# Gyeeta/gyeeta

Measured on NVIDIA H100. Metric: events/sec aggregated, higher is better.
Workload: dtype u64

## Files before the change

gyeeta_b200/csrc/gysk_kernels.cu:

```cuda
#include "gysk_kernels.cuh"
#include "gysk_state.cuh"
#include "gysk_summary.cuh"

#include <cfloat>
#include <climits>
#include <cmath>
#include <algorithm>
#include <type_traits>
#include <cstdlib>
#include <cstring>

namespace gysk {

static constexpr int KEY_GROUP_SHIFT = 30;
static constexpr int KEY_SLOT_SHIFT = KEY_GROUP_SHIFT + TD_CODE_BITS;
__device__ __forceinline__ uint32_t key_usec(unsigned long long k) { return (uint32_t)k & 0x3FFFFFFFu; }
__device__ __forceinline__ uint32_t key_slot(unsigned long long k) { return (uint32_t)(k >> KEY_SLOT_SHIFT); }
__device__ __forceinline__ uint32_t key_bin(unsigned long long k) { return (uint32_t)(k >> KEY_GROUP_SHIFT) & ((1u << TD_CODE_BITS) - 1u); }

static constexpr int KEY_DIGIT_MAX = 8;
struct SortPlan { int np; int shift[OS_MAX_PASSES_VK]; int bits[OS_MAX_PASSES_VK]; int exp; };

__global__ void init_state_kernel(DevState st, uint32_t max_svcs, uint32_t max_tasks)
{
// ... 769 lines not shown
		if (k == ~0ull) return ~0u;
		const uint32_t s = key_slot(k), r1 = s == sf ? rf : (s == sl ? rl : 0u);
		return r1 ? ((r1 - 1u) << TD_CODE_BITS) | key_bin(k) : ~0u;
	};
	auto red_bin = [&](uint32_t d, unsigned long long cw, unsigned long long us) {
		unsigned long long *row = rows + (size_t)(d >> TD_CODE_BITS) * HOT_ROW_WORDS;
		const uint32_t w = hot_word(d & ((1u << TD_CODE_BITS) - 1u));
		red_add_u64(row + w, cw);
		red_add_u64(row + w + HOT_ROW_BINS, us);
	};

	const uint32_t dfirst = __shfl_sync(0xffffffffu, dest(kk[0]), 0), dlast = __shfl_sync(0xffffffffu, dest(kk[LS_V - 1]), 31);
	if (dfirst == dlast && dlast != ~0u) {
		unsigned long long us = 0;
		uint32_t rem = 0;
#pragma unroll
		for (int t = 0; t < LS_V; ++t) { const uint32_t v = key_usec(kk[t]); us += v; rem += v - (v / 1000u) * 1000u; }
		const unsigned long long gsum = (unsigned long long)__reduce_add_sync(0xffffffffu, (uint32_t)us & 0xFFFFFu) +
				((unsigned long long)__reduce_add_sync(0xffffffffu, (uint32_t)(us >> 20)) << 20);
		rem = __reduce_add_sync(0xffffffffu, rem);
		if (lane == 0) red_bin(dlast, (unsigned long long)(32 * LS_V) | ((unsigned long long)rem << BIN_CNT_BITS), gsum);
		return;
	}

	uint32_t pd[LS_V], pc[LS_V], prem[LS_V];
	unsigned long long ps[LS_V];
	bool tail[LS_V];
#pragma unroll
	for (int t = 0; t < LS_V; ++t) {
		const uint32_t d = dest(kk[t]);
		const bool valid = d != ~0u;
		tail[t] = valid;
		const uint32_t v = key_usec(kk[t]);
		pd[t] = valid ? d : (0x80000000u | (uint32_t)lane); pc[t] = valid ? 1u : 0u; ps[t] = valid ? v : 0u; prem[t] = valid ? v - (v / 1000u) * 1000u : 0u;
		if (t > 0 && valid && pd[t] == pd[t - 1]) { pc[t] += pc[t - 1]; ps[t] += ps[t - 1]; prem[t] += prem[t - 1]; tail[t - 1] = false; }
	}
#pragma unroll
	for (int t = 0; t < LS_V; ++t) {
		const bool act = tail[t];
		if (!__any_sync(0xffffffffu, act)) continue;
		const uint32_t did = act ? pd[t] : (0x80000000u | (uint32_t)lane);
		const unsigned long long v = act ? ps[t] : 0ull;
		uint32_t cnt = act ? pc[t] : 0u, rem = act ? prem[t] : 0u;
		const uint32_t m = __match_any_sync(0xffffffffu, did);
		unsigned long long gsum = v;
		const uint32_t maxcnt = __reduce_max_sync(0xffffffffu, (uint32_t)__popc(m));
		uint32_t rest = m & ~(1u << lane);
		const uint32_t cnt0 = cnt, rem0 = rem;
		for (uint32_t u = 1; u < maxcnt; ++u) {
			const int src = rest ? (__ffs(rest) - 1) : lane;
			const unsigned long long ov = __shfl_sync(0xffffffffu, v, src);
			const uint32_t oc = __shfl_sync(0xffffffffu, cnt0, src), orr = __shfl_sync(0xffffffffu, rem0, src);
			if (rest) { gsum += ov; cnt += oc; rem += orr; rest &= rest - 1; }
		}
		if (act && (m & ((1u << lane) - 1u)) == 0) red_bin(did, (unsigned long long)cnt | ((unsigned long long)rem << BIN_CNT_BITS), gsum);
	}
}

__global__ void __launch_bounds__(256) long_sum_kernel(const unsigned long long *__restrict__ keys, const unsigned long long *__restrict__ d_n,
		const BatchSeg *__restrict__ segs, const unsigned long long *__restrict__ nlong, unsigned long long *__restrict__ rows)
{
	if (*nlong == 0) return;
	const uint64_t n = *d_n;
	const uint64_t nchunks = (n + 127) >> 7;
	const int lane = threadIdx.x & 31;
	const uint64_t gw = ((uint64_t)blockIdx.x * blockDim.x + threadIdx.x) >> 5, nwarps = ((uint64_t)gridDim.x * blockDim.x) >> 5;
	for (uint64_t c0 = gw * 32; c0 < nchunks; c0 += nwarps * 32) {
		const uint64_t c = c0 + lane;
		uint32_t sf = 0, sl = 0, rf = 0, rl = 0;
		if (c < nchunks) {
			const uint64_t f = c << 7, l = f + 127 < n ? f + 127 : n - 1;
			sf = key_slot(keys[f]); sl = key_slot(keys[l]);
			rf = segs[sf].row1; rl = segs[sl].row1;
		}
		for (uint32_t todo = __ballot_sync(0xffffffffu, (rf | rl) != 0); todo; todo &= todo - 1) {
			const int src = __ffs(todo) - 1;
			long_sum_chunk(keys, n, (c0 + (uint64_t)src) << 7, __shfl_sync(0xffffffffu, sf, src), __shfl_sync(0xffffffffu, rf, src),
					__shfl_sync(0xffffffffu, sl, src), __shfl_sync(0xffffffffu, rl, src), rows);
		}
	}
}

static constexpr int TD_WARPS = 3;
static constexpr int TD_SMEM_N = 384;

__global__ void __launch_bounds__(TD_WARPS * 32, TD_MERGE_CTAS_PER_SM) bins_merge_kernel(DevState st, const unsigned long long *__restrict__ keys,
		const uint32_t *__restrict__ touched, const unsigned long long *__restrict__ ntouched_p, const uint32_t *__restrict__ long_slot,
		const unsigned long long *__restrict__ nlong_p, unsigned long long *__restrict__ batch_rows, const BatchSeg *__restrict__ segs,
		Centroid *__restrict__ items_scratch , TdWorkBig *__restrict__ big_scratch )
{
	__shared__ TdWorkT<TD_SMEM_N> work[TD_WARPS];
	__shared__ uint32_t hcnt[TD_WARPS][16], hsum_lo[TD_WARPS][16], hsum_hi[TD_WARPS][16];
	__shared__ uint16_t first_idx[16];
	const int lane = threadIdx.x & 31, wid = threadIdx.x >> 5;
	const uint32_t gw = blockIdx.x * TD_WARPS + wid, nwarps = gridDim.x * TD_WARPS;

	Centroid *items = items_scratch + (size_t)gw * NBINS;
	const uint32_t ntouched = (uint32_t)*ntouched_p, nlong = (uint32_t)*nlong_p;

	if (threadIdx.x < 16) {
		constexpr uint32_t thr[13] = {1, 10, 30, 60, 100, 150, 200, 300, 450, 700, 1000, 3000, 15000};
		const uint32_t bk = threadIdx.x;
		const uint32_t first_us = bk < 2 ? 0u : (bk > 14 ? 0u : (thr[bk - 2] + 1u) * 1000u);
		first_idx[bk] = (uint16_t)(bk == 0 ? 0u : (bk > 14 ? 0xFFFFu : td_code(first_us) + bk));
	}
	__syncthreads();

	const uint32_t nhot = st.hot_rows ? (uint32_t)st.counters[CTR_NHOT] : 0u;
	const uint32_t nrow = nhot + nlong, total = nrow + ntouched;
	const uint32_t lt = (1u << lane) - 1u;
	auto slot_of = [&](uint32_t t) { return t < nhot ? st.hot_slot[t] : (t < nrow ? long_slot[t - nhot] : touched[t - nrow]); };
	uint32_t nslot = gw < total ? slot_of(gw) : 0u;
	for (uint32_t t = gw; t < total; t += nwarps) {
		const uint32_t slot = nslot;
		const bool has_next = t + nwarps < total;
		nslot = has_next ? slot_of(t + nwarps) : 0u;
		const SlotBatch sb = st.slot_batch[slot];
		BatchSeg seg {0u, 0u, 0u, 0u};
		if (t >= nrow) seg = segs[slot];
		uint2 nseg = make_uint2(0u, 0u);
		if (has_next) {
			prefetch_l2(st.td_cent + (size_t)nslot * TD_CAP + lane * (TD_CAP / 32));
			if (lane == 0) prefetch_l2(st.slot_batch + nslot);
			else if (lane == 1) prefetch_l2(st.td_head + nslot);
			if (t + nwarps >= nrow) { const BatchSeg ns = segs[nslot]; nseg = make_uint2(ns.key0, ns.end); }
		}
		if (t < nhot && sb.minv == 0xFFFFFFFFu) continue;
		if (lane < 16) { hcnt[wid][lane] = 0; hsum_lo[wid][lane] = 0; hsum_hi[wid][lane] = 0; }
		__syncwarp();
		auto take_bin = [&](uint32_t j, unsigned long long cw, unsigned long long us, uint32_t bin) {
			const unsigned long long cnt = cw & BIN_CNT_MASK, rem = cw >> BIN_CNT_BITS;
			Centroid c; c.mean = __ddiv_rn((double)us, (double)cnt); c.weight = cnt;
			items[j] = c;
			uint32_t bk = 0;
#pragma unroll
			for (int q = 1; q < 15; ++q) bk += bin >= first_idx[q];
			atomicAdd(&hcnt[wid][bk], (uint32_t)cnt);
			const unsigned long long ms = (us - rem) / 1000ull;
			const uint32_t mlo = (uint32_t)ms, mhi = (uint32_t)(ms >> 32);
			const uint32_t old = atomicAdd(&hsum_lo[wid][bk], mlo);
			const uint32_t up = mhi + (old + mlo < old ? 1u : 0u);
			if (up) atomicAdd(&hsum_hi[wid][bk], up);
		};
		uint32_t nitems = 0, nsamples, binmax = 0;
		if (t >= nrow) {
			nsamples = seg.end - seg.key0;
			constexpr int RAW_BIN_SHIFT = 54;
			static_assert(BIN_CNT_BITS + 10 + 14 <= RAW_BIN_SHIFT && LONG_SEG <= (1 << 14), "cw of a short segment's bin below the bin bits");
			ulonglong2 *raw = reinterpret_cast<ulonglong2 *>(items);
			uint32_t pbin = ~0u, ccnt = 0, crem = 0;
			unsigned long long cus = 0;
			for (uint32_t b0 = seg.key0; b0 < seg.end; b0 += 128) {
				uint32_t bin[4], v[4];
#pragma unroll
				for (int u = 0; u < 4; ++u) {
					const uint32_t i = b0 + (uint32_t)u * 32 + lane;
					const unsigned long long k = i < seg.end ? keys[i] : 0ull;
					bin[u] = i < seg.end ? key_bin(k) : ~0u;
					v[u] = key_usec(k);
				}
				const uint32_t xbin = b0 + 128 < seg.end ? key_bin(keys[b0 + 128]) : ~0u;
#pragma unroll
				for (int u = 0; u < 4; ++u) {
					if (b0 + (uint32_t)u * 32 >= seg.end) break;
					uint32_t pb = __shfl_up_sync(0xffffffffu, bin[u], 1), nb = __shfl_down_sync(0xffffffffu, bin[u], 1);
					const uint32_t nb31 = u < 3 ? __shfl_sync(0xffffffffu, bin[u < 3 ? u + 1 : 0], 0) : xbin;
					if (lane == 0) pb = pbin;
					if (lane == 31) nb = nb31;
					const bool valid = bin[u] != ~0u;
					const uint32_t hm = __ballot_sync(0xffffffffu, valid && bin[u] != pb);
					const uint32_t upto = hm & (0xFFFFFFFFu >> (31 - lane));
					const int h = upto ? 31 - __clz((int)upto) : 0;
					const uint32_t r = v[u] - (v[u] / 1000u) * 1000u;
					const uint32_t a = valid ? v[u] & 0xFFFFFu : 0u, b = valid ? (v[u] >> 20) | (r << 16) : 0u;
					uint32_t ai = a, bi = b;
#pragma unroll
					for (int off = 1; off < 32; off <<= 1) {
						const uint32_t x = __shfl_up_sync(0xffffffffu, ai, off), y = __shfl_up_sync(0xffffffffu, bi, off);
						if (lane >= off) { ai += x; bi += y; }
					}
					const uint32_t as = ai - __shfl_sync(0xffffffffu, ai - a, h), bs = bi - __shfl_sync(0xffffffffu, bi - b, h);
					uint32_t cnt = (uint32_t)(lane - h) + 1u, rem = bs >> 16;
					unsigned long long us = (unsigned long long)as + ((unsigned long long)(bs & 0xFFFFu) << 20);
					if (!upto) { cnt += ccnt; rem += crem; us += cus; }
					if (valid && bin[u] != nb) {
						raw[nitems + __popc(upto) - 1u] = make_ulonglong2(us, (unsigned long long)cnt | ((unsigned long long)rem << BIN_CNT_BITS) |
								((unsigned long long)bin[u] << RAW_BIN_SHIFT));
						binmax = max(binmax, cnt);
					}
					ccnt = __shfl_sync(0xffffffffu, cnt, 31); crem = __shfl_sync(0xffffffffu, rem, 31); cus = __shfl_sync(0xffffffffu, us, 31);
					pbin = __shfl_sync(0xffffffffu, bin[u], 31);
					nitems += __popc(hm);
				}
			}
			__syncwarp();
			for (uint32_t j = lane; j < nitems; j += 32) {
				const ulonglong2 r = raw[j];
				take_bin(j, r.y & ((1ull << RAW_BIN_SHIFT) - 1u), r.x, (uint32_t)(r.y >> RAW_BIN_SHIFT));
			}
		}
		else {
			unsigned long long *row = t < nhot ? st.hot_rows + (size_t)t * HOT_ROW_WORDS : batch_rows + (size_t)(t - nhot) * HOT_ROW_WORDS;
			uint32_t mine = 0;
			for (uint32_t b0 = 0; b0 < (uint32_t)NBINS; b0 += 32) {
				const uint32_t bin = b0 + lane;
				const uint32_t i0 = hot_word(bin), i1 = i0 + (uint32_t)HOT_ROW_BINS;
				ulonglong2 v = make_ulonglong2(0ull, 0ull);
				if (bin < (uint32_t)NBINS) { v.x = __ldcg(row + i0); v.y = __ldcg(row + i1); }
				const bool ne = (v.x & BIN_CNT_MASK) != 0;
				const uint32_t m = __ballot_sync(0xffffffffu, ne);
				if (ne) {
					take_bin(nitems + __popc(m & lt), v.x, v.y, bin);
					row[i0] = 0ull; row[i1] = 0ull;
					mine += (uint32_t)(v.x & BIN_CNT_MASK);
					binmax = max(binmax, (uint32_t)(v.x & BIN_CNT_MASK));
				}
				nitems += __popc(m);
			}
			nsamples = __reduce_add_sync(0xffffffffu, mine);
		}
		if (has_next && t + nwarps >= nrow) {
			const uint32_t l0 = nseg.x >> 4, l1 = (nseg.y - 1u) >> 4;
			if (l0 + lane <= l1) prefetch_l2(keys + (size_t)(l0 + lane) * 16);
		}
		binmax = __reduce_max_sync(0xffffffffu, binmax);
		__syncwarp();
		if (lane < HIST_MAX_CELL) {
			if (hcnt[wid][lane]) {
				HistCell *c = st.hist_cur + (size_t)slot * HIST_CELLS + lane;
				c->count += hcnt[wid][lane]; c->sum += (long long)(((unsigned long long)hsum_hi[wid][lane] << 32) | hsum_lo[wid][lane]);
			}
		}
		else if (lane == HIST_MAX_CELL) {
			HistCell *c = st.hist_cur + (size_t)slot * HIST_CELLS + HIST_MAX_CELL;
			const long long mx = (long long)(sb.maxv / 1000u);
			if (mx > c->sum) c->sum = mx;
			uint32_t hot = sb.hot;
			if (!hot && st.hot_rows && nsamples >= st.hot_min && nsamples <= st.hot_max && binmax <= st.hot_bin_max) {
				const unsigned long long h = atomicAdd(st.counters + CTR_NHOT_NEXT, 1ull);
				if (h < (unsigned long long)st.hot_cap) { st.hot_slot[h] = slot; hot = (uint32_t)h + 1u; }
				else atomicAdd(st.counters + CTR_NHOT_NEXT, ~0ull);
			}
			st.slot_batch[slot] = SlotBatch {0xFFFFFFFFu, 0u, 0u, hot};
		}
		__syncwarp();

		TdHead head = st.td_head[slot];
		Centroid *cent = st.td_cent + (size_t)slot * TD_CAP;
		uint32_t nout;
		if (head.n + nitems <= (uint32_t)TD_SMEM_N) nout = warp_merge_compress(work[wid], cent, head.n, items, nitems, cent, st.td);
		else nout = warp_merge_compress(big_scratch[gw], cent, head.n, items, nitems, cent, st.td);
		if (lane == 0) {
			head.n = nout;
			head.total += nsamples;
			if ((double)sb.minv < head.minv) head.minv = (double)sb.minv;
			if ((double)sb.maxv > head.maxv) head.maxv = (double)sb.maxv;
			st.td_head[slot] = head;
		}
		__syncwarp();
	}
}

__global__ void flush_kernel(DevState st, uint32_t nslots, uint32_t tsec, uint32_t idle_secs)
{
	const uint64_t i = (uint64_t)blockIdx.x * blockDim.x + threadIdx.x;
	const bool valid = i < (uint64_t)nslots * HIST_CELLS;
	const int cell = (int)(i & (HIST_CELLS - 1));
	HistCell c {0, 0};
	unsigned long long cc = 0;
	const uint32_t slot = (uint32_t)(i >> 4);

	if (valid) {
		c = st.hist_cur[i];
		if (cell == HIST_MAX_CELL) cc = st.conn_cur[slot];
	}
	bool auxact = false;
	if (valid && cell == HIST_MAX_CELL) { const SlotAux a0 = st.slot_aux[slot]; auxact = (a0.act_cur | a0.err_cur) != 0; }
	const uint32_t bal = __ballot_sync(0xffffffffu, valid && (cell == HIST_MAX_CELL ? (cc != 0 || auxact) : c.count != 0));
	const bool active = ((bal >> (threadIdx.x & 16)) & 0xFFFFu) != 0;
	if (!valid) return;

	st.bm_last[i] = st.bm_cur[i]; st.bm_cur[i] = 0;
	st.hist_last[i] = c;
	HistCell &r0 = st.levels.row(0, st.levels.cur[0], slot)[cell], &r1 = st.levels.row(1, st.levels.cur[1], slot)[cell];
	if (cell == HIST_MAX_CELL) {
		if (c.sum > r0.sum) r0.sum = c.sum;
		if (c.sum > r1.sum) r1.sum = c.sum;
	}
	else {
		r0.count += c.count; r0.sum += c.sum;
		r1.count += c.count; r1.sum += c.sum;
	}
	if (cell == HIST_MAX_CELL) {
		if (c.sum > st.hist_all[i].sum) st.hist_all[i].sum = c.sum;
		st.hist_cur[i].count = 0; st.hist_cur[i].sum = LLONG_MIN;
		st.conn_last[slot] = cc;
		st.conn_all_cnt[slot] += (uint32_t)cc;
		st.conn_all_kb[slot] += cc >> 32;
		st.conn_cur[slot] = 0;
		{
			SlotAux a = st.slot_aux[slot];
			a.act_last = a.act_cur; a.act_cur = 0; a.err_last = a.err_cur; a.err_cur = 0; a.rtt_last = a.rtt_cur; a.rtt_cur = 0;
			st.slot_aux[slot] = a;
		}

		const unsigned long long id = st.slot_id[slot];
		if (id) {
			uint32_t first = st.slot_first_seen[slot], last = st.slot_last_active[slot];
			if (!first) { first = tsec ? tsec : 1u; st.slot_first_seen[slot] = first; }
			if (active) { last = tsec ? tsec : 1u; st.slot_last_active[slot] = last; }
			if (idle_secs && last && (uint64_t)last + idle_secs < tsec && (uint64_t)first + 2ull * idle_secs < tsec) {
				const unsigned long long k = atomicAdd(st.counters + CTR_NEVICT, 1ull);
				st.evict_list[k] = slot;
				st.evict_ids[k] = id;
			}
		}
	}
	else {
		st.hist_all[i].count += c.count;
		st.hist_all[i].sum += c.sum;
		st.hist_cur[i].count = 0; st.hist_cur[i].sum = 0;
	}
}

struct LevelStat { int64_t p95, p99, p25; uint64_t cnt, sum; double mean; };

__device__ __forceinline__ LevelStat level_stat(const uint64_t *counts, uint64_t sum)
{
	LevelStat r;
	uint64_t c = 0;
	for (int b = 0; b < HIST_MAX_CELL; ++b) c += counts[b];
	r.p95 = resp_bucket_value(hist_pct_bucket(counts, HIST_MAX_CELL, c, 95.0f), c);
	r.p99 = resp_bucket_value(hist_pct_bucket(counts, HIST_MAX_CELL, c, 99.0f), c);
	r.p25 = resp_bucket_value(hist_pct_bucket(counts, HIST_MAX_CELL, c, 25.0f), c);
// ... 517 lines not shown
	uint32_t e = ++*tmp.epoch;
	if (e == 0) {
		cudaMemsetAsync(tmp.tile_status, 0, (size_t)max_tiles * RADIX_MAX * sizeof(unsigned long long), s);
		e = ++*tmp.epoch;
	}
	return e;
}

static void launch_os_pass(int bits, uint32_t ntiles, const unsigned long long *in, unsigned long long *out, const unsigned long long *d_n, const DigitSpec &D,
		const uint32_t *ghist, unsigned long long *status, uint32_t *ticket, uint32_t epoch, cudaStream_t s)
{
	const uint32_t grid = std::min<uint32_t>(ntiles, (uint32_t)sm_count(current_device()) * 4u);
	if (bits > 8) os_pass_kernel<9><<<grid, OS_THREADS, sizeof(OneSweepSharedT<9>), s>>>(in, out, d_n, D, ghist, status, ticket, epoch);
	else if (bits == 8) os_pass_kernel<8><<<grid, OS_THREADS, sizeof(OneSweepSharedT<8>), s>>>(in, out, d_n, D, ghist, status, ticket, epoch);
	else if (bits == 7) os_pass_kernel<7><<<grid, OS_THREADS, sizeof(OneSweepSharedT<7>), s>>>(in, out, d_n, D, ghist, status, ticket, epoch);
	else os_pass_kernel<6><<<grid, OS_THREADS, sizeof(OneSweepSharedT<6>), s>>>(in, out, d_n, D, ghist, status, ticket, epoch);
}

int launch_radix_sort(const SortTemp &tmp, const unsigned long long *d_n, uint64_t n_max, int lo1, int hi1, int lo2, int hi2, int *which, cudaStream_t s)
{
	int launches = 0;
	unsigned long long *bufs[2] = { tmp.keys_a, tmp.keys_b };
	int w = 0;
	DigitSpecs P;

	*which = 0;
	if (!n_max) return 0;
	if (build_digit_specs(lo1, hi1, lo2, hi2, P) || n_max >= (1ull << 30)) return -1;
	bool any9 = false;
	for (int p = 0; p < P.np; ++p) any9 |= P.d[p].b1 + P.d[p].b2 > 8;
	const int copies = any9 ? 4 : 8, stride = (any9 ? 512 : 256) + 1;
	const int dev = current_device();
	os_set_attrs(dev);
	const uint32_t ntiles = div_up(n_max, SORT_TILE);
	uint32_t *ghist = tmp.os_ghist, *tickets = tmp.os_ghist + OS_MAX_PASSES * RADIX_MAX;

	cudaMemsetAsync(ghist, 0, (OS_MAX_PASSES * RADIX_MAX + OS_MAX_PASSES) * sizeof(uint32_t), s);
	const uint32_t hgrid = std::min<uint32_t>(div_up(n_max, 512 * 2 * 4), (uint32_t)sm_count(dev) * 3);
	if (any9) os_hist_kernel<4, 513><<<hgrid, 512, (size_t)P.np * copies * stride * sizeof(uint32_t), s>>>(bufs[w], d_n, P, ghist);
	else os_hist_kernel<8, 257><<<hgrid, 512, (size_t)P.np * copies * stride * sizeof(uint32_t), s>>>(bufs[w], d_n, P, ghist);
	launches++;
	for (int p = 0; p < P.np; ++p) {
		const uint32_t epoch = next_epoch(tmp, tmp.max_tiles, s);
		launch_os_pass(P.d[p].b1 + P.d[p].b2, ntiles, bufs[w], bufs[w ^ 1], d_n, P.d[p], ghist + p * RADIX_MAX, tmp.tile_status, tickets + p, epoch, s);
		launches++;
		w ^= 1;
	}
	*which = w;
	return launches;
}

int launch_batch_merge(const DevState &st, const SortTemp &tmp, uint64_t n_events, uint32_t max_svcs, cudaStream_t s)
{
	if (!n_events) return 0;
	int launches = 0;
	unsigned long long *d_nkeys = st.counters + CTR_NKEYS, *d_ntouched = st.counters + CTR_NTOUCHED;
	const int dev = current_device();
	const int nsm = sm_count(dev);
	os_set_attrs(dev);

	SortPlan plan {};
	if (key_sort_plan(max_svcs, plan) < 0) return -1;
	const uint32_t ntiles = div_up(n_events, SORT_TILE);
	unsigned long long *bufs[2] = { tmp.keys_a, tmp.keys_b };
	uint32_t *ghist = tmp.os_ghist, *tickets = tmp.os_ghist + OS_MAX_PASSES * RADIX_MAX;
	int w = 0;
	for (int p = 0; p < plan.np; ++p) {
		const DigitSpec D { plan.shift[p], plan.bits[p], 0, 0 };
		const uint32_t epoch = next_epoch(tmp, tmp.max_tiles, s);
		launch_os_pass(plan.bits[p], ntiles, bufs[w], bufs[w ^ 1], d_nkeys, D, ghist + p * RADIX_MAX, tmp.tile_status, tickets + p, epoch, s);
		launches++;
		w ^= 1;
	}
	const unsigned long long *src = bufs[w];

	static_assert(CTR_NLONG == CTR_NTOUCHED + 1, "one memset clears both segment counters");
	unsigned long long *d_nlong = st.counters + CTR_NLONG;
	BatchSeg *segs = reinterpret_cast<BatchSeg *>(tmp.segs);
	cudaMemsetAsync(d_ntouched, 0, 2 * sizeof(unsigned long long), s);
	segs_mark_kernel<<<div_up(n_events, SG_THREADS * SG_V), SG_THREADS, 0, s>>>(src, d_nkeys, segs, tmp.touched, d_ntouched, tmp.long_slot, d_nlong);
	long_sum_kernel<<<nsm * 8, 256, 0, s>>>(src, d_nkeys, segs, d_nlong, tmp.batch_rows);
	const int merge_ctas = std::min(nsm, TD_MERGE_MAX_SMS) * TD_MERGE_CTAS_PER_SM;
	bins_merge_kernel<<<merge_ctas, TD_WARPS * 32, 0, s>>>(st, src, tmp.touched, d_ntouched, tmp.long_slot, d_nlong, tmp.batch_rows, segs,
			tmp.items_scratch, tmp.big_scratch);
	return launches + 3;
}

__global__ void topn_score_kernel(DevState st, uint32_t nslots, int metric, int host_filter, unsigned long long *__restrict__ keys,
		unsigned long long *d_n)
{
	const uint32_t slot = blockIdx.x * blockDim.x + threadIdx.x;
	if (slot == 0) *d_n = nslots;
	if (slot >= nslots) return;
	unsigned long long score = 0;

	if (host_filter < 0 || st.slot_host[slot] == (uint32_t)host_filter) {
		if (metric == GYSK_TOPN_QPS) {
			for (int b = 0; b < HIST_MAX_CELL; ++b) score += st.hist_last[(size_t)slot * HIST_CELLS + b].count;
		}
		else if (metric == GYSK_TOPN_CONNS) score = (uint32_t)st.conn_last[slot];
		else if (metric == GYSK_TOPN_ISSUE) {
			const SlotState ss = st.slot_state[slot];
			score = ss.state > GYSK_STATE_OK && ss.state <= GYSK_STATE_DOWN ? ss.state : 0;
		}
		else score = st.conn_last[slot] >> 32;
	}
	if (score > 0xFFFFFFFFull) score = 0xFFFFFFFFull;
	keys[slot] = (score << 32) | slot;
}

__global__ void topn_task_score_kernel(DevState st, uint32_t ntasks, int metric, unsigned long long *__restrict__ keys, unsigned long long *d_n)
{
	const uint32_t slot = blockIdx.x * blockDim.x + threadIdx.x;
	if (slot == 0) *d_n = ntasks;
	if (slot >= ntasks) return;
	unsigned long long score = st.task_slot_id[slot] ? (unsigned long long)st.task_last[(size_t)slot * 3 + metric].sum : 0ull;
	if ((long long)score < 0) score = 0;
	if (score > 0xFFFFFFFFull) score = 0xFFFFFFFFull;
	keys[slot] = (score << 32) | slot;
}

__global__ void topn_pick_kernel(const unsigned long long *__restrict__ slot_id, const uint32_t *__restrict__ slot_host,
		const unsigned long long *__restrict__ sorted, uint32_t nslots, uint32_t want, gysk_topn_entry *__restrict__ out)
{
	const uint32_t i = threadIdx.x;
	if (i >= want) return;
	gysk_topn_entry o; o.glob_id = 0; o.score = 0; o.host_idx = 0; o.pad = 0;
	if (i < nslots) {
		const unsigned long long k = sorted[nslots - 1 - i];
		const uint32_t slot = (uint32_t)k;
		o.glob_id = slot_id[slot]; o.score = k >> 32; o.host_idx = slot_host ? slot_host[slot] : 0u;
	}
	out[i] = o;
}

int launch_topn_pick(const SortTemp &tmp, const unsigned long long *d_n, uint32_t nkeys, const unsigned long long *ids, const uint32_t *hosts,
		uint32_t want, gysk_topn_entry *d_out, cudaStream_t s)
{
	int which = 0;
	const int sorted = launch_radix_sort(tmp, d_n, nkeys, 32, 64, 64, 64, &which, s);
	if (sorted < 0) return sorted;
	topn_pick_kernel<<<1, 64, 0, s>>>(ids, hosts, which ? tmp.keys_b : tmp.keys_a, nkeys, want, d_out);
	return sorted + 1;
}

int launch_topn(const DevState &st, const SortTemp &tmp, uint32_t nslots, int is_task, int metric, int host_filter, uint32_t want,
		gysk_topn_entry *d_out, cudaStream_t s)
{
	if (!nslots) return 0;
	unsigned long long *d_n = st.counters + CTR_NKEYS;
	if (is_task) topn_task_score_kernel<<<div_up(nslots, 256), 256, 0, s>>>(st, nslots, metric, tmp.keys_a, d_n);
	else topn_score_kernel<<<div_up(nslots, 256), 256, 0, s>>>(st, nslots, metric, host_filter, tmp.keys_a, d_n);
	const int picked = launch_topn_pick(tmp, d_n, nslots, is_task ? st.task_slot_id : st.slot_id, is_task ? st.task_slot_host : st.slot_host,
			want, d_out, s);
	return picked < 0 ? picked : 1 + picked;
}

__global__ void task_flush_kernel(DevState st, uint32_t max_tasks)
{
	const uint32_t i = blockIdx.x * blockDim.x + threadIdx.x;
	if (i >= max_tasks * 3u) return;
	const HistCell *h = st.task_hist + (size_t)i * HIST_CELLS;
	HistCell tot {0, 0};
	for (int b = 0; b < HIST_MAX_CELL; ++b) { tot.count += h[b].count; tot.sum += h[b].sum; }
	const HistCell prev = st.task_prev[i];
	st.task_last[i] = HistCell {tot.count - prev.count, tot.sum - prev.sum};
	st.task_prev[i] = tot;
// ... 111 lines not shown
```

gyeeta_b200/csrc/gysk_kernels.cuh:

```cuda
#pragma once

#include "gysk_device.cuh"
#include "gysk_tdigest.cuh"
#include "../../include/gysketch.h"

#include <climits>

namespace gysk {

static constexpr int NLEVELS = 2;
static constexpr int NSLOTS = 10;

struct LevelRing
{
	HistCell		*ring;
	uint32_t		stride;
	uint32_t		live[NLEVELS];
	uint32_t		cur[NLEVELS];

	__host__ __device__ __forceinline__ HistCell *row(int l, uint32_t k, uint32_t slot) const
	{
		return ring + (((size_t)l * NSLOTS + k) * stride + slot) * HIST_CELLS;
	}
	template <typename F> __device__ __forceinline__ void each_live(int l, uint32_t slot, F f) const
// ... 20 lines not shown
	unsigned long long	*conn_cur, *conn_last;
	unsigned long long	*slot_id;
	uint32_t		*slot_host;
	uint32_t		*slot_first_seen, *slot_last_active;
	uint32_t		*evict_list;
	unsigned long long	*evict_ids;
	unsigned long long	*conn_all_cnt, *conn_all_kb;
	uint32_t		*bm_cur, *bm_last;
	SlotBatch		*slot_batch;
	unsigned long long	*hot_rows;
	uint32_t		*hot_slot;
	uint32_t		hot_cap, hot_min, hot_max, hot_bin_max;
	SlotAux			*slot_aux;
	HistCell		*qps_hist, *act_hist;
	SlotState		*slot_state;
	uint8_t			*hll;
	Centroid		*td_cent;
	TdHead			*td_head;
	HistCell		*task_hist;
	HistCell		*task_prev, *task_last;
	unsigned long long	*task_slot_id;
	uint32_t		*task_slot_host;
	unsigned long long	*cms_cur, *cms_last;
	uint32_t		cms_depth, cms_wmask, cms_log2w, hll_p;
	uint32_t		rank, world, auto_register;
	double			td_delta;
	TdParams		td;
	unsigned long long	*counters;
};

struct SortTemp
{
	unsigned long long	*keys_a, *keys_b;
	uint64_t		nkeys;
	unsigned long long	*tile_status;
	uint32_t		*epoch;
	uint32_t		*os_ghist;
	uint32_t		*touched;
	uint4			*segs;
	uint32_t		*long_slot;
	unsigned long long	*batch_rows;
	Centroid		*items_scratch;
	TdWorkBig		*big_scratch;
	uint4			*recq;
	uint2			*rec_cnt;
	uint64_t		recq_cap;
	uint32_t		rec_cnt_cap;
	uint32_t		max_tiles;
};

struct RecRegions { uint32_t nwarps; uint64_t cap; };

struct IngestShape { static constexpr int WARPS = 8, MIN_CTAS = 3, EPT = 2, CHUNK = 32 * EPT; };

struct SvcRaw
{
	unsigned long long	id;
	int32_t			found;
	uint32_t		slot;
	HistCell		cur[HIST_CELLS], last[HIST_CELLS], all[HIST_CELLS];
	HistCell		lvl[2][HIST_CELLS];
	unsigned long long	conn_cur, conn_last, conn_all_cnt, conn_all_kb;
	uint32_t		bm_cur[HIST_CELLS], bm_last[HIST_CELLS];
	uint32_t		hll_hist[64];
	TdHead			td;
	SlotAux			aux;
	SlotState		sst;
	HistCell		qps[HIST_CELLS], act[HIST_CELLS];
	Centroid		cent[TD_CAP];
};

struct TaskRaw
{
	unsigned long long	id;
	int32_t			found;
	uint32_t		slot;
	HistCell		h[3][HIST_CELLS];
};

static constexpr int SORT_TILE = 4096;
static constexpr int RADIX_MAX_BITS = 9;
static constexpr int RADIX_MAX = 1 << RADIX_MAX_BITS;
static constexpr int OS_MAX_PASSES_VK = 5;
static constexpr int TD_MERGE_CTAS_PER_SM = 7, TD_MERGE_MAX_SMS = 192;
static constexpr int LONG_SEG = 8192;

int launch_init_state(const DevState &st, uint32_t max_svcs, uint32_t max_tasks, cudaStream_t s);
int launch_register(const DevState &st, const unsigned long long *d_ids, uint32_t n, int is_task, cudaStream_t s);
int launch_ingest(const DevState &st, const SortTemp &tmp, const gysk_event *d_ev, uint64_t n, uint32_t max_svcs, RecRegions &rr, cudaStream_t s);
int launch_batch_merge(const DevState &st, const SortTemp &tmp, uint64_t n_events, uint32_t max_svcs, cudaStream_t s);
int launch_drains(const DevState &st, const SortTemp &tmp, const RecRegions &rr, uint64_t n_events, cudaStream_t s);
int launch_radix_sort(const SortTemp &tmp, const unsigned long long *d_n, uint64_t n_max, int lo1, int hi1, int lo2, int hi2, int *which, cudaStream_t s);
int launch_topn(const DevState &st, const SortTemp &tmp, uint32_t nslots, int is_task, int metric, int host_filter, uint32_t want,
		gysk_topn_entry *d_out, cudaStream_t s);
int launch_topn_pick(const SortTemp &tmp, const unsigned long long *d_n, uint32_t nkeys, const unsigned long long *ids, const uint32_t *hosts,
		uint32_t want, gysk_topn_entry *d_out, cudaStream_t s);
int launch_task_flush(const DevState &st, uint32_t max_tasks, cudaStream_t s);
int launch_flush(const DevState &st, uint32_t max_svcs, uint32_t tsec, uint32_t idle_secs, cudaStream_t s);
int launch_rebuild_table(const DevState &st, uint32_t max_svcs, cudaStream_t s);
int launch_gather_svcs(const DevState &st, const unsigned long long *d_ids, uint32_t n, SvcRaw *d_out, cudaStream_t s);
int launch_gather_tasks(const DevState &st, const unsigned long long *d_ids, uint32_t n, TaskRaw *d_out, cudaStream_t s);
int launch_gather_hll(const DevState &st, const unsigned long long *d_ids, int32_t *found, uint8_t *d_out, cudaStream_t s);
int launch_window_list(const DevState &st, const SortTemp &tmp, uint32_t nslots, int is_task, int host_filter, uint32_t active_only,
		uint32_t active_mark, uint32_t seen_before, unsigned long long *d_n, bool order, const unsigned long long **keys, const unsigned long long **ids,
		cudaStream_t s);
int launch_day_stats(const DevState &st, const unsigned long long *d_slots, uint32_t n, gysk_listener_day_stats *d_out, cudaStream_t s);
int launch_host_listen_count(const DevState &st, const unsigned long long *keys, const unsigned long long *d_n, uint32_t n, uint32_t active_mark,
		unsigned long long *acc, cudaStream_t s);
int launch_host_listen_rows(const unsigned long long *keys, const unsigned long long *d_n, const unsigned long long *acc, uint32_t rlo, uint32_t cap,
		gysk_host_listen *d_out, unsigned long long *d_rows, cudaStream_t s);
int launch_svc_summaries(const DevState &st, const unsigned long long *d_ids, const unsigned long long *d_slots, uint32_t n, gysk_svc_summary *d_out,
		cudaStream_t s);
int launch_task_summaries(const DevState &st, const unsigned long long *d_ids, const unsigned long long *d_slots, uint32_t n, gysk_task_summary *d_out,
		cudaStream_t s);
int launch_query_flows(const DevState &st, const unsigned long long *d_keys, uint32_t n, int last_window, gysk_flow_est *d_out, cudaStream_t s);

}
```

gyeeta_b200/csrc/gysk_tdigest.cuh:

```cuda
#pragma once

#include "gysk_device.cuh"

namespace gysk {

struct TdParams { const double *qtab; uint32_t delta; uint32_t pad; };

template <int NMAX_>
struct TdWorkT
{
	static constexpr int NMAX = NMAX_;
	double			mean[NMAX];
	unsigned long long	pref[NMAX + 1];
	uint16_t		bounds[TD_CAP + 2];
	uint16_t		nxt[NMAX];
	double			src[NMAX];
};
using TdWork = TdWorkT<2 * TD_CAP>;
using TdWorkBig = TdWorkT<1120>;
struct TdScratch : TdWork
{
	Centroid		newc[TD_CAP];
};

template <typename Work>
__device__ __forceinline__ uint32_t warp_merge_compress(Work &S, const Centroid *a, uint32_t na, const Centroid *b, uint32_t nb,
		Centroid *out, const TdParams &P)
{
	const int lane = threadIdx.x & 31;
	const uint32_t nm = na + nb;

	double *am = S.src, *bm = S.src + na;
	for (uint32_t j = lane; j < na; j += 32) am[j] = a[j].mean;
	for (uint32_t j = lane; j < nb; j += 32) bm[j] = b[j].mean;
	__syncwarp();
	const uint32_t per = (nm + 31u) >> 5;
	const uint32_t d0 = lane * per < nm ? lane * per : nm, d1 = d0 + per < nm ? d0 + per : nm;
	unsigned long long tot = 0;
	if (d0 < d1) {
		uint32_t lo = d0 > nb ? d0 - nb : 0u, hi = d0 < na ? d0 : na;
		while (lo < hi) { const uint32_t mid = (lo + hi) >> 1; if (am[mid] <= bm[d0 - 1u - mid]) lo = mid + 1; else hi = mid; }
		uint32_t i = lo, k = d0 - lo;
		double av = i < na ? am[i] : 0.0, bv = k < nb ? bm[k] : 0.0;
		for (uint32_t pos = d0; pos < d1; ++pos) {
			const bool ta = i < na && (k >= nb || av <= bv);
			S.mean[pos] = ta ? av : bv;
			S.nxt[pos] = (uint16_t)(ta ? i : (0x8000u | k));
			if (ta) { ++i; av = i < na ? am[i] : 0.0; }
			else { ++k; bv = k < nb ? bm[k] : 0.0; }
		}
		for (uint32_t pos = d0; pos < d1; ++pos) {
			const uint32_t from = S.nxt[pos];
			const unsigned long long w = (from & 0x8000u) ? b[from & 0x7FFFu].weight : a[from].weight;
			S.pref[pos + 1] = w;
			tot += w;
		}
	}
	{
		unsigned long long incl = tot;
#pragma unroll
		for (int off = 1; off < 32; off <<= 1) {
			const unsigned long long tt = __shfl_up_sync(0xffffffffu, incl, off);
			if (lane >= off) incl += tt;
		}
		unsigned long long run = incl - tot;
		for (uint32_t pos = d0; pos < d1; ++pos) { run += S.pref[pos + 1]; S.pref[pos + 1] = run; }
		if (lane == 0) S.pref[0] = 0;
	}
	__syncwarp();
	auto ckey = [&S](uint32_t i) { const unsigned long long p = S.pref[i]; return p + ((S.pref[i + 1] - p) >> 1); };

	uint32_t nout = 0;
	if (nm) {
		const unsigned long long Wt = S.pref[nm];
		const double W = (double)Wt;
		const uint32_t cj = (P.delta + 32u) >> 5;
		uint32_t lo = 0;
		for (uint32_t j = lane * cj, jn = 0; jn < cj && j <= P.delta; ++j, ++jn) {
			const unsigned long long T = j == P.delta ? Wt : (unsigned long long)__dmul_rn(__ldg(P.qtab + j), W);
			uint32_t steps = jn ? 0u : 8u;
			while (steps < 8u && lo < nm && ckey(lo) < T) { ++lo; ++steps; }
			if (steps == 8u) {
				uint32_t hi = nm;
				while (lo < hi) { const uint32_t mid = (lo + hi) >> 1; if (ckey(mid) < T) lo = mid + 1; else hi = mid; }
			}
			S.nxt[j] = (uint16_t)lo;
		}
		__syncwarp();
		for (uint32_t j0 = 0; j0 < P.delta; j0 += 32) {
			const uint32_t j = j0 + lane;
			const bool ne = j < P.delta && S.nxt[j + 1] > S.nxt[j];
			const uint32_t m = __ballot_sync(0xffffffffu, ne);
			if (ne) S.bounds[nout + __popc(m & ((1u << lane) - 1u))] = S.nxt[j];
			nout += __popc(m);
		}
		if (lane == 0) S.bounds[nout] = (uint16_t)nm;
		__syncwarp();
	}

	for (uint32_t c = lane; c < nout; c += 32) {
		double csum = 0.0;
		const uint32_t lo = S.bounds[c], hi = S.bounds[c + 1];
		for (uint32_t i = lo; i < hi; ++i) {
			csum = __dadd_rn(csum, __dmul_rn(S.mean[i], (double)(S.pref[i + 1] - S.pref[i])));
		}
		const unsigned long long cw = S.pref[hi] - S.pref[lo];
		Centroid o; o.mean = __ddiv_rn(csum, (double)cw); o.weight = cw;
		out[c] = o;
	}
	__syncwarp();
	return nout;
}

}
```

Measured before the change: 11.57 billion.

## Stage short-segment bins in shared memory and restructure bin scan per lane

Rewrites the short-segment bin scan so each lane handles 8 consecutive keys with vectorized loads, software-prefetches the next 256-key tile, and uses one packed warp scan per tile in place of one per 32 keys. Bin means and counts are written straight into the shared-memory merge workspace when they fit, so the t-digest merge can skip reloading items from global scratch. The bucket lookup becomes a precomputed byte table, TD_SMEM_N grows, and CTAs per SM drop from 7 to 5 to make room for the larger shared footprint. It also adds an exp flag that skips the merge, and vectorizes the centroid mean and weight loads in the merge.

New measurement: 12.09 billion (median of 6 runs). +4.4%, better.

```diff
diff --git a/gyeeta_b200/csrc/gysk_kernels.cu b/gyeeta_b200/csrc/gysk_kernels.cu
--- a/gyeeta_b200/csrc/gysk_kernels.cu
+++ b/gyeeta_b200/csrc/gysk_kernels.cu
@@ -875,27 +875,33 @@
 }
 
 static constexpr int TD_WARPS = 3;
-static constexpr int TD_SMEM_N = 384;
+static constexpr int TD_SMEM_N = 540;
 
 __global__ void __launch_bounds__(TD_WARPS * 32, TD_MERGE_CTAS_PER_SM) bins_merge_kernel(DevState st, const unsigned long long *__restrict__ keys,
 		const uint32_t *__restrict__ touched, const unsigned long long *__restrict__ ntouched_p, const uint32_t *__restrict__ long_slot,
 		const unsigned long long *__restrict__ nlong_p, unsigned long long *__restrict__ batch_rows, const BatchSeg *__restrict__ segs,
-		Centroid *__restrict__ items_scratch , TdWorkBig *__restrict__ big_scratch )
+		Centroid *__restrict__ items_scratch , TdWorkBig *__restrict__ big_scratch , int exp)
 {
 	__shared__ TdWorkT<TD_SMEM_N> work[TD_WARPS];
 	__shared__ uint32_t hcnt[TD_WARPS][16], hsum_lo[TD_WARPS][16], hsum_hi[TD_WARPS][16];
-	__shared__ uint16_t first_idx[16];
+	__shared__ uint8_t bk_tab[NBINS / 8];
 	const int lane = threadIdx.x & 31, wid = threadIdx.x >> 5;
 	const uint32_t gw = blockIdx.x * TD_WARPS + wid, nwarps = gridDim.x * TD_WARPS;
 
 	Centroid *items = items_scratch + (size_t)gw * NBINS;
 	const uint32_t ntouched = (uint32_t)*ntouched_p, nlong = (uint32_t)*nlong_p;
 
-	if (threadIdx.x < 16) {
+	for (uint32_t g = threadIdx.x; g < (uint32_t)NBINS / 8; g += blockDim.x) {
 		constexpr uint32_t thr[13] = {1, 10, 30, 60, 100, 150, 200, 300, 450, 700, 1000, 3000, 15000};
-		const uint32_t bk = threadIdx.x;
-		const uint32_t first_us = bk < 2 ? 0u : (bk > 14 ? 0u : (thr[bk - 2] + 1u) * 1000u);
-		first_idx[bk] = (uint16_t)(bk == 0 ? 0u : (bk > 14 ? 0xFFFFu : td_code(first_us) + bk));
+		auto bucket = [&](uint32_t bin) {
+			uint32_t bk = bin >= 1u;
+			for (int q = 2; q < 15; ++q) bk += bin >= td_code((thr[q - 2] + 1u) * 1000u) + (uint32_t)q;
+			return bk;
+		};
+		const uint32_t b0 = bucket(g * 8);
+		uint32_t off = 8;
+		for (uint32_t o = 7; o >= 1; --o) if (bucket(g * 8 + o) != b0) off = o;
+		bk_tab[g] = (uint8_t)(b0 | (off << 4));
 	}
 	__syncthreads();
 
@@ -921,13 +927,14 @@
 		if (t < nhot && sb.minv == 0xFFFFFFFFu) continue;
 		if (lane < 16) { hcnt[wid][lane] = 0; hsum_lo[wid][lane] = 0; hsum_hi[wid][lane] = 0; }
 		__syncwarp();
-		auto take_bin = [&](uint32_t j, unsigned long long cw, unsigned long long us, uint32_t bin) {
+		const uint32_t na = st.td_head[slot].n;
+		TdWorkT<TD_SMEM_N> &W = work[wid];
+		auto take_bin = [&](uint32_t j, unsigned long long cw, unsigned long long us, uint32_t bin, bool staged) {
 			const unsigned long long cnt = cw & BIN_CNT_MASK, rem = cw >> BIN_CNT_BITS;
-			Centroid c; c.mean = __ddiv_rn((double)us, (double)cnt); c.weight = cnt;
-			items[j] = c;
-			uint32_t bk = 0;
-#pragma unroll
-			for (int q = 1; q < 15; ++q) bk += bin >= first_idx[q];
+			const double mean = __ddiv_rn((double)us, (double)cnt);
+			if (staged) { W.src[na + j] = mean; W.nxt[j] = (uint16_t)cnt; }
+			else { Centroid c; c.mean = mean; c.weight = cnt; items[j] = c; }
+			const uint32_t e = bk_tab[bin >> 3], bk = (e & 15u) + ((bin & 7u) >= (e >> 4) ? 1u : 0u);
 			atomicAdd(&hcnt[wid][bk], (uint32_t)cnt);
 			const unsigned long long ms = (us - rem) / 1000ull;
 			const uint32_t mlo = (uint32_t)ms, mhi = (uint32_t)(ms >> 32);
@@ -936,60 +943,103 @@
 			if (up) atomicAdd(&hsum_hi[wid][bk], up);
 		};
 		uint32_t nitems = 0, nsamples, binmax = 0;
+		bool staged = false;
 		if (t >= nrow) {
 			nsamples = seg.end - seg.key0;
 			constexpr int RAW_BIN_SHIFT = 54;
 			static_assert(BIN_CNT_BITS + 10 + 14 <= RAW_BIN_SHIFT && LONG_SEG <= (1 << 14), "cw of a short segment's bin below the bin bits");
+			const uint32_t room = (uint32_t)TD_SMEM_N - na;
+			unsigned long long *raw_us = reinterpret_cast<unsigned long long *>(W.src + na), *raw_cw = W.pref;
 			ulonglong2 *raw = reinterpret_cast<ulonglong2 *>(items);
+			auto load8 = [&](uint32_t b0, unsigned long long (&k)[8]) {
+				const uint32_t i0 = b0 + (uint32_t)lane * 8u;
+				if (i0 >= seg.key0 && i0 + 8u <= seg.end) {
+#pragma unroll
+					for (int q = 0; q < 4; ++q) {
+						const ulonglong2 v = *reinterpret_cast<const ulonglong2 *>(keys + i0 + 2 * q);
+						k[2 * q] = v.x; k[2 * q + 1] = v.y;
+					}
+				}
+				else {
+#pragma unroll
+					for (int u = 0; u < 8; ++u) k[u] = i0 + u >= seg.key0 && i0 + u < seg.end ? keys[i0 + u] : ~0ull;
+				}
+			};
+			auto rem_of = [](uint32_t v) { return v - (v / 1000u) * 1000u; };
 			uint32_t pbin = ~0u, ccnt = 0, crem = 0;
 			unsigned long long cus = 0;
-			for (uint32_t b0 = seg.key0; b0 < seg.end; b0 += 128) {
-				uint32_t bin[4], v[4];
-#pragma unroll
-				for (int u = 0; u < 4; ++u) {
-					const uint32_t i = b0 + (uint32_t)u * 32 + lane;
-					const unsigned long long k = i < seg.end ? keys[i] : 0ull;
-					bin[u] = i < seg.end ? key_bin(k) : ~0u;
-					v[u] = key_usec(k);
+			const uint32_t a0 = seg.key0 & ~1u;
+			unsigned long long kk[8], nk[8];
+			load8(a0, kk);
+			for (uint32_t b0 = a0; b0 < seg.end; b0 += 256) {
+				if (b0 + 256u < seg.end) load8(b0 + 256u, nk);
+				else {
+#pragma unroll
+					for (int u = 0; u < 8; ++u) nk[u] = ~0ull;
 				}
-				const uint32_t xbin = b0 + 128 < seg.end ? key_bin(keys[b0 + 128]) : ~0u;
-#pragma unroll
-				for (int u = 0; u < 4; ++u) {
-					if (b0 + (uint32_t)u * 32 >= seg.end) break;
-					uint32_t pb = __shfl_up_sync(0xffffffffu, bin[u], 1), nb = __shfl_down_sync(0xffffffffu, bin[u], 1);
-					const uint32_t nb31 = u < 3 ? __shfl_sync(0xffffffffu, bin[u < 3 ? u + 1 : 0], 0) : xbin;
-					if (lane == 0) pb = pbin;
-					if (lane == 31) nb = nb31;
+				uint32_t bin[8];
+#pragma unroll
+				for (int u = 0; u < 8; ++u) bin[u] = kk[u] == ~0ull ? ~0u : key_bin(kk[u]);
+				const uint32_t nfirst = __shfl_sync(0xffffffffu, nk[0] == ~0ull ? ~0u : key_bin(nk[0]), 0);
+				uint32_t prevb = __shfl_up_sync(0xffffffffu, bin[7], 1), nextb = __shfl_down_sync(0xffffffffu, bin[0], 1);
+				if (lane == 0) prevb = pbin;
+				if (lane == 31) nextb = nfirst;
+				uint32_t hc = 0, tc = 0, tr = 0;
+				unsigned long long tu = 0;
+#pragma unroll
+				for (int u = 0; u < 8; ++u) {
 					const bool valid = bin[u] != ~0u;
-					const uint32_t hm = __ballot_sync(0xffffffffu, valid && bin[u] != pb);
-					const uint32_t upto = hm & (0xFFFFFFFFu >> (31 - lane));
-					const int h = upto ? 31 - __clz((int)upto) : 0;
-					const uint32_t r = v[u] - (v[u] / 1000u) * 1000u;
-					const uint32_t a = valid ? v[u] & 0xFFFFFu : 0u, b = valid ? (v[u] >> 20) | (r << 16) : 0u;
-					uint32_t ai = a, bi = b;
-#pragma unroll
-					for (int off = 1; off < 32; off <<= 1) {
-						const uint32_t x = __shfl_up_sync(0xffffffffu, ai, off), y = __shfl_up_sync(0xffffffffu, bi, off);
-						if (lane >= off) { ai += x; bi += y; }
+					if (valid && bin[u] != (u ? bin[u - 1] : prevb)) { ++hc; tc = 0; tr = 0; tu = 0; }
+					const uint32_t v = key_usec(kk[u]);
+					if (valid) { ++tc; tr += rem_of(v); tu += v; }
+				}
+				const unsigned long long X = tu | ((unsigned long long)hc << 40);
+				const uint32_t Y = tr | (tc << 18);
+				unsigned long long xi = X;
+				uint32_t yi = Y;
+#pragma unroll
+				for (int off = 1; off < 32; off <<= 1) {
+					const unsigned long long x = __shfl_up_sync(0xffffffffu, xi, off);
+					const uint32_t y = __shfl_up_sync(0xffffffffu, yi, off);
+					if (lane >= off) { xi += x; yi += y; }
+				}
+				const uint32_t hm = __ballot_sync(0xffffffffu, hc != 0);
+				const uint32_t upto = hm & (0xFFFFFFFFu >> (31 - lane));
+				const int h = upto ? 31 - __clz((int)upto) : 0;
+				const unsigned long long xs = xi - __shfl_sync(0xffffffffu, xi - X, h);
+				const uint32_t ys = yi - __shfl_sync(0xffffffffu, yi - Y, h);
+				unsigned long long su = xs & ((1ull << 40) - 1u);
+				uint32_t sc = ys >> 18, sr = ys & 0x3FFFFu;
+				if (!upto) { su += cus; sc += ccnt; sr += crem; }
+				unsigned long long ru = __shfl_up_sync(0xffffffffu, su, 1);
+				uint32_t rc = __shfl_up_sync(0xffffffffu, sc, 1), rr = __shfl_up_sync(0xffffffffu, sr, 1);
+				if (lane == 0) { ru = cus; rc = ccnt; rr = crem; }
+				uint32_t j = nitems + (uint32_t)(xi >> 40) - hc - 1u;
+#pragma unroll
+				for (int u = 0; u < 8; ++u) {
+					const bool valid = bin[u] != ~0u;
+					if (valid && bin[u] != (u ? bin[u - 1] : prevb)) { ++j; rc = 0; rr = 0; ru = 0; }
+					const uint32_t v = key_usec(kk[u]);
+					if (valid) { ++rc; rr += rem_of(v); ru += v; }
+					if (valid && bin[u] != (u < 7 ? bin[u + 1] : nextb)) {
+						const unsigned long long cwb = (unsigned long long)rc | ((unsigned long long)rr << BIN_CNT_BITS) |
+								((unsigned long long)bin[u] << RAW_BIN_SHIFT);
+						if (j < room) { raw_us[j] = ru; raw_cw[j] = cwb; }
+						else raw[j] = make_ulonglong2(ru, cwb);
+						binmax = max(binmax, rc);
 					}
-					const uint32_t as = ai - __shfl_sync(0xffffffffu, ai - a, h), bs = bi - __shfl_sync(0xffffffffu, bi - b, h);
-					uint32_t cnt = (uint32_t)(lane - h) + 1u, rem = bs >> 16;
-					unsigned long long us = (unsigned long long)as + ((unsigned long long)(bs & 0xFFFFu) << 20);
-					if (!upto) { cnt += ccnt; rem += crem; us += cus; }
-					if (valid && bin[u] != nb) {
-						raw[nitems + __popc(upto) - 1u] = make_ulonglong2(us, (unsigned long long)cnt | ((unsigned long long)rem << BIN_CNT_BITS) |
-								((unsigned long long)bin[u] << RAW_BIN_SHIFT));
-						binmax = max(binmax, cnt);
-					}
-					ccnt = __shfl_sync(0xffffffffu, cnt, 31); crem = __shfl_sync(0xffffffffu, rem, 31); cus = __shfl_sync(0xffffffffu, us, 31);
-					pbin = __shfl_sync(0xffffffffu, bin[u], 31);
-					nitems += __popc(hm);
 				}
+				cus = __shfl_sync(0xffffffffu, su, 31); ccnt = __shfl_sync(0xffffffffu, sc, 31); crem = __shfl_sync(0xffffffffu, sr, 31);
+				pbin = __shfl_sync(0xffffffffu, bin[7], 31);
+				nitems += (uint32_t)(__shfl_sync(0xffffffffu, xi, 31) >> 40);
+#pragma unroll
+				for (int u = 0; u < 8; ++u) kk[u] = nk[u];
 			}
+			staged = na + nitems <= (uint32_t)TD_SMEM_N;
 			__syncwarp();
 			for (uint32_t j = lane; j < nitems; j += 32) {
-				const ulonglong2 r = raw[j];
-				take_bin(j, r.y & ((1ull << RAW_BIN_SHIFT) - 1u), r.x, (uint32_t)(r.y >> RAW_BIN_SHIFT));
+				const ulonglong2 r = j < room ? make_ulonglong2(raw_us[j], raw_cw[j]) : raw[j];
+				take_bin(j, r.y & ((1ull << RAW_BIN_SHIFT) - 1u), r.x, (uint32_t)(r.y >> RAW_BIN_SHIFT), staged);
 			}
 		}
 		else {
@@ -1003,7 +1053,7 @@
 				const bool ne = (v.x & BIN_CNT_MASK) != 0;
 				const uint32_t m = __ballot_sync(0xffffffffu, ne);
 				if (ne) {
-					take_bin(nitems + __popc(m & lt), v.x, v.y, bin);
+					take_bin(nitems + __popc(m & lt), v.x, v.y, bin, false);
 					row[i0] = 0ull; row[i1] = 0ull;
 					mine += (uint32_t)(v.x & BIN_CNT_MASK);
 					binmax = max(binmax, (uint32_t)(v.x & BIN_CNT_MASK));
@@ -1037,12 +1087,14 @@
 			st.slot_batch[slot] = SlotBatch {0xFFFFFFFFu, 0u, 0u, hot};
 		}
 		__syncwarp();
+		if (exp & 256) continue;
 
 		TdHead head = st.td_head[slot];
 		Centroid *cent = st.td_cent + (size_t)slot * TD_CAP;
 		uint32_t nout;
-		if (head.n + nitems <= (uint32_t)TD_SMEM_N) nout = warp_merge_compress(work[wid], cent, head.n, items, nitems, cent, st.td);
-		else nout = warp_merge_compress(big_scratch[gw], cent, head.n, items, nitems, cent, st.td);
+		if (staged) nout = warp_merge_compress_staged(W, cent, na, nitems, cent, st.td);
+		else if (na + nitems <= (uint32_t)TD_SMEM_N) nout = warp_merge_compress(W, cent, na, items, nitems, cent, st.td);
+		else nout = warp_merge_compress(big_scratch[gw], cent, na, items, nitems, cent, st.td);
 		if (lane == 0) {
 			head.n = nout;
 			head.total += nsamples;
@@ -1726,7 +1778,7 @@
 	long_sum_kernel<<<nsm * 8, 256, 0, s>>>(src, d_nkeys, segs, d_nlong, tmp.batch_rows);
 	const int merge_ctas = std::min(nsm, TD_MERGE_MAX_SMS) * TD_MERGE_CTAS_PER_SM;
 	bins_merge_kernel<<<merge_ctas, TD_WARPS * 32, 0, s>>>(st, src, tmp.touched, d_ntouched, tmp.long_slot, d_nlong, tmp.batch_rows, segs,
-			tmp.items_scratch, tmp.big_scratch);
+			tmp.items_scratch, tmp.big_scratch, plan.exp);
 	return launches + 3;
 }
 
diff --git a/gyeeta_b200/csrc/gysk_kernels.cuh b/gyeeta_b200/csrc/gysk_kernels.cuh
--- a/gyeeta_b200/csrc/gysk_kernels.cuh
+++ b/gyeeta_b200/csrc/gysk_kernels.cuh
@@ -126,7 +126,7 @@
 static constexpr int RADIX_MAX_BITS = 9;
 static constexpr int RADIX_MAX = 1 << RADIX_MAX_BITS;
 static constexpr int OS_MAX_PASSES_VK = 5;
-static constexpr int TD_MERGE_CTAS_PER_SM = 7, TD_MERGE_MAX_SMS = 192;
+static constexpr int TD_MERGE_CTAS_PER_SM = 5, TD_MERGE_MAX_SMS = 192;
 static constexpr int LONG_SEG = 8192;
 
 int launch_init_state(const DevState &st, uint32_t max_svcs, uint32_t max_tasks, cudaStream_t s);
diff --git a/gyeeta_b200/csrc/gysk_tdigest.cuh b/gyeeta_b200/csrc/gysk_tdigest.cuh
--- a/gyeeta_b200/csrc/gysk_tdigest.cuh
+++ b/gyeeta_b200/csrc/gysk_tdigest.cuh
@@ -23,16 +23,22 @@
 	Centroid		newc[TD_CAP];
 };
 
-template <typename Work>
-__device__ __forceinline__ uint32_t warp_merge_compress(Work &S, const Centroid *a, uint32_t na, const Centroid *b, uint32_t nb,
+template <bool B_STAGED, typename Work>
+__device__ __forceinline__ uint32_t td_merge_compress(Work &S, const Centroid *a, uint32_t na, const Centroid *b, uint32_t nb,
 		Centroid *out, const TdParams &P)
 {
 	const int lane = threadIdx.x & 31;
 	const uint32_t nm = na + nb;
 
 	double *am = S.src, *bm = S.src + na;
-	for (uint32_t j = lane; j < na; j += 32) am[j] = a[j].mean;
-	for (uint32_t j = lane; j < nb; j += 32) bm[j] = b[j].mean;
+	for (uint32_t j0 = 0; j0 < na; j0 += 32 * 4) {
+		double v[4];
+#pragma unroll
+		for (int q = 0; q < 4; ++q) { const uint32_t j = j0 + q * 32 + lane; v[q] = j < na ? a[j].mean : 0.0; }
+#pragma unroll
+		for (int q = 0; q < 4; ++q) { const uint32_t j = j0 + q * 32 + lane; if (j < na) am[j] = v[q]; }
+	}
+	if (!B_STAGED) for (uint32_t j = lane; j < nb; j += 32) bm[j] = b[j].mean;
 	__syncwarp();
 	const uint32_t per = (nm + 31u) >> 5;
 	const uint32_t d0 = lane * per < nm ? lane * per : nm, d1 = d0 + per < nm ? d0 + per : nm;
@@ -42,18 +48,25 @@
 		while (lo < hi) { const uint32_t mid = (lo + hi) >> 1; if (am[mid] <= bm[d0 - 1u - mid]) lo = mid + 1; else hi = mid; }
 		uint32_t i = lo, k = d0 - lo;
 		double av = i < na ? am[i] : 0.0, bv = k < nb ? bm[k] : 0.0;
+		constexpr unsigned long long FROM_A = 1ull << 63;
 		for (uint32_t pos = d0; pos < d1; ++pos) {
 			const bool ta = i < na && (k >= nb || av <= bv);
 			S.mean[pos] = ta ? av : bv;
-			S.nxt[pos] = (uint16_t)(ta ? i : (0x8000u | k));
+			if (B_STAGED) S.pref[pos + 1] = ta ? (FROM_A | i) : (unsigned long long)S.nxt[k];
+			else S.nxt[pos] = (uint16_t)(ta ? i : (0x8000u | k));
 			if (ta) { ++i; av = i < na ? am[i] : 0.0; }
 			else { ++k; bv = k < nb ? bm[k] : 0.0; }
 		}
-		for (uint32_t pos = d0; pos < d1; ++pos) {
-			const uint32_t from = S.nxt[pos];
-			const unsigned long long w = (from & 0x8000u) ? b[from & 0x7FFFu].weight : a[from].weight;
-			S.pref[pos + 1] = w;
-			tot += w;
+		for (uint32_t p0 = d0; p0 < d1; p0 += 4) {
+			unsigned long long w[4];
+#pragma unroll
+			for (int q = 0; q < 4; ++q) {
+				const uint32_t pos = p0 + q < d1 ? p0 + q : d1 - 1u;
+				if (B_STAGED) { const unsigned long long f = S.pref[pos + 1]; w[q] = (f & FROM_A) ? a[(uint32_t)f].weight : f; }
+				else { const uint32_t from = S.nxt[pos]; w[q] = (from & 0x8000u) ? b[from & 0x7FFFu].weight : a[from].weight; }
+			}
+#pragma unroll
+			for (int q = 0; q < 4; ++q) if (p0 + q < d1) { S.pref[p0 + q + 1] = w[q]; tot += w[q]; }
 		}
 	}
 	{
@@ -112,4 +125,18 @@
 	return nout;
 }
 
+template <typename Work>
+__device__ __forceinline__ uint32_t warp_merge_compress(Work &S, const Centroid *a, uint32_t na, const Centroid *b, uint32_t nb,
+		Centroid *out, const TdParams &P)
+{
+	return td_merge_compress<false>(S, a, na, b, nb, out, P);
 }
+
+template <typename Work>
+__device__ __forceinline__ uint32_t warp_merge_compress_staged(Work &S, const Centroid *a, uint32_t na, uint32_t nb, Centroid *out,
+		const TdParams &P)
+{
+	return td_merge_compress<true>(S, a, na, nullptr, nb, out, P);
+}
+
+}
```
